# xiexh20/VisTracker

Hardware: AMD Instinct MI355X
Metric: frames/sec joint SMPL+object fit (higher is better)
Workload: dtype f32 (decoder GEMMs: 22-bit split-f16 operands x3 MFMA, fp32 accumulate)

## Files before the change

### include/vistracker.h

```cpp
#ifndef VISTRACKER_H
#define VISTRACKER_H

#ifdef __cplusplus
extern "C" {
#endif

#define VT_OK 0
#define VT_ERR_ARG -1
#define VT_ERR_HIP -2
#define VT_ERR_BUSY -3

#define VT_SMPL_V 6890
#define VT_SMPL_J 52
#define VT_SMPL_NB 10
#define VT_SMPL_NP 459
#define VT_FEAT 611
#define VT_HID 128

const char *vt_last_error(void);
int vt_version(void);

typedef struct vt_smplh vt_smplh;

int vt_smplh_create(vt_smplh **out, const float *v_template, const float *shapedirs, const float *posedirs,
// ... 153 lines not shown

int vt_sqdiff_loss(const float *a, int a_stride, const float *b, int b_stride, int rows, int cols, float denom,
                   float gscale, double *term, float *da, void *stream);

long vt_collision_workspace_bytes(int B, int n_smpl_faces);
int vt_collision_loss(const float *smpl_verts, int n_smpl_verts, const int *smpl_faces, int n_smpl_faces, const float *obj_verts, int n_obj_verts,
                      const int *obj_faces, int n_obj_faces, int B, float sigma, int max_collisions, float gscale, double *term,
                      float *d_obj_t, int *pairs_per_frame, void *workspace, void *stream);

int vt_chamfer_ragged(const float *x, const int *offx, const float *y, const int *offy, int P, float gscale,
                      double *term, float *dx, float *dy, void *stream);
long vt_chamfer_ws_bytes(long total_x, long total_y, int P);
int vt_chamfer_ragged_ws(const float *x, const int *offx, long total_x, const float *y, const int *offy, long total_y, int P, float gscale,
                         double *term, float *dx, float *dy, void *ws, void *stream);

int vt_chamfer_ragged_idx(const float *x, const int *offx, long total_x, const float *y_base, const int *idx_y, const int *offy, long total_y, int P,
                          float gscale, double *term, float *dy_base, void *ws, int run_plan, void *stream);

int vt_nn_distance(const float *query, int nq, const float *search, int ns, int P, float *dist, void *stream);

long vt_sil_workspace_floats(int B, int NV, int NF, int size);
int vt_sil_forward(const float *verts, int B, int NV, const int *faces, int NF, const float *K, int size,
                   float *image, int *face_index, float *ws, void *stream);
int vt_sil_backward(const float *verts, int B, int NV, const int *faces, int NF, const float *K, int size,
                    const int *face_index, const float *d_image, float eps, float *ws, float *dverts, void *stream);
int vt_sil_setup(const float *mask_h, const float *mask_o, int B, int H, int W, const float *crop_centers, double expansion, int out, double crop_size,
                 double net_size, const double *cam_norm, double image_width, float *image_ref, float *keep_mask, float *K, double *boxes_ws, void *stream);

int vt_sil_mask_loss(const float *image, const float *keep, const float *ref, const float *occ, int B, int size,
                     float gscale, double *term, float *per_frame, float *d_image, void *stream);

int vt_sil_step(const float *verts, int B, int NV, const int *faces, int NF, const float *K, int size, const float *keep, const float *ref,
                const float *occ, float gscale, float eps, double *term, int *face_index, float *d_image, float *ws, float *dverts, void *stream);

int vt_triplane_render(const float *verts, const float *center, int B, int NV, const int *faces, int NF, int size,
                       float *masks, int *face_index, float *ws, void *stream);

int vt_upsample2x_bicubic_add(const float *low, const float *skip, int B, int h, int w, int C, float *out, void *stream);
int vt_upsample2x_bicubic_add_stats(const float *low, const float *skip, int B, int h, int w, int C, float *out, double *stats_ws, int stats_groups,
                                    void *stream);

long vt_groupnorm_workspace_doubles(int B, int HW, int C, int groups);
int vt_groupnorm_nhwc(const float *x, const float *gamma, const float *beta, int B, int HW, int C, int groups, float eps,
                      int relu, double *ws, float *y, void *stream);

int vt_adam_step(float *p, const float *g, float *m, float *v, long n, int step, float lr, float beta1, float beta2,
                 float eps, const int *stop_flag, void *stream);

int vt_adam_step_2d(float *p, long p_stride, const float *g, long g_stride, float *m, float *v, int rows, int cols,
                    int step, float lr, float beta1, float beta2, float eps, const int *stop_flag, void *stream);

int vt_loss_reduce_and_stop(const double *terms, const float *w, int nterms, float tol, int armed, float *state,
                            int *stop_flag, float *history, int slot, void *stream);

int vt_fill(float *p, long n, float value, void *stream);

int vt_stream_set_skip_flag(void *stream, const int *flag);

int vt_gen_round_compact(const float *surface, const float *df_target, const float *pre, const unsigned char *active, int B, int S, float filter_val,
                         float zmin, const long long *fill, int cap, int write, float *buf_points, int *order, float *kept_pre, long long *cnt,
                         long long *fill_out, void *stream);
int vt_gen_scatter_heads(const float *pred, int B, int C, int kmax, const long long *fill_old, const long long *cnt, int cap, float *buf, void *stream);
int vt_gen_resample(const float *samples, const int *order, const long long *cnt, const float *init, int B, int S, int S0, const float *u,
                    const float *pert, int M, float near_scale, float *out, void *stream);

long vt_render_workspace_bytes(int B, int NF, int size, int anti_aliasing, long list_entries);
// ... 49 lines not shown
```

### vistracker_amd/_lib.py

```python
from __future__ import annotations

import ctypes as C
import os

_HERE = os.path.dirname(os.path.abspath(__file__))
LIB_PATH = os.environ.get("VT_LIB_PATH", os.path.join(_HERE, "libvistracker_hip.so"))

vp = C.c_void_p
fp = C.c_void_p
ci = C.c_int
cl = C.c_long
cf = C.c_float
cd = C.c_double


class VtMaps(C.Structure):
    _fields_ = [("maps", C.c_void_p * 8), ("res", C.c_int * 8), ("proj", C.c_void_p), ("proj_cols", C.c_int),
                ("act_level", C.c_int), ("proj_level", C.c_int), ("force_fp32", C.c_int)]


SIGNATURES = {
    "vt_last_error": (C.c_char_p, []),
    "vt_version": (ci, []),
    "vt_smplh_create": (ci, [C.POINTER(vp), vp, vp, vp, vp, vp, vp, vp]),
# ... 53 lines not shown
    "vt_conv1x1_destroy": (None, [vp]),
    "vt_conv1x1_forward": (ci, [vp, fp, ci, ci, fp, fp, fp, ci, ci, ci, ci, fp, ci, ci, fp, ci, ci, fp, ci, vp]),
    "vt_conv3x3_forward_block": (ci, [vp, fp, ci, ci, fp, fp, fp, ci, ci, ci, ci, fp, ci, ci, fp, ci, ci, fp, ci, ci, fp, ci, vp]),
    "vt_conv3x3_forward_block_stats": (ci, [vp, fp, ci, ci, fp, fp, fp, ci, ci, ci, ci, fp, ci, ci, fp, ci, ci, fp, ci, ci, fp, ci, fp, ci, vp]),
    "vt_avgpool2x2_stats": (ci, [fp, ci, ci, ci, ci, fp, fp, ci, vp]),
    "vt_sweep_blocks": (ci, [ci]),
    "vt_upsample2x_bicubic_add_stats": (ci, [fp, fp, ci, ci, ci, ci, fp, fp, ci, vp]),
    "vt_conv3x3_forward_gn_stats": (ci, [vp, fp, ci, ci, fp, fp, fp, ci, ci, ci, ci, fp, ci, ci, fp, ci, vp]),
    "vt_triplane_render": (ci, [fp, fp, ci, ci, fp, ci, ci, fp, fp, fp, vp]),
    "vt_query_project_step": (ci, [vp, C.POINTER(VtMaps), fp, fp, fp, ci, ci, ci, cf, fp, fp, vp]),
    "vt_query_projection_floats": (C.c_long, [C.POINTER(VtMaps), ci]),
    "vt_query_build_projection": (ci, [vp, C.POINTER(VtMaps), ci, fp, vp]),
    "vt_so3_project_forward": (ci, [fp, fp, ci, fp, vp]),
    "vt_so3_project_backward": (ci, [fp, fp, ci, fp, fp, vp]),
    "vt_rigid_forward": (ci, [fp, ci, fp, fp, fp, ci, ci, fp, vp]),
    "vt_rigid_backward": (ci, [fp, ci, fp, ci, ci, fp, fp, fp, ci, vp]),
    "vt_accel_loss": (ci, [fp, ci, ci, fp, cf, fp, fp, vp]),
    "vt_accel_loss_strided": (ci, [fp, ci, ci, ci, fp, cf, fp, fp, vp]),
    "vt_velocity_loss": (ci, [fp, ci, ci, cf, fp, fp, vp]),
    "vt_kpts_loss": (ci, [fp, fp, fp, ci, ci, ci, vp, cf, cf, fp, fp, vp]),
    "vt_sqdiff_loss": (ci, [fp, ci, fp, ci, ci, ci, cf, cf, fp, fp, vp]),
    "vt_chamfer_ragged": (ci, [fp, fp, fp, fp, ci, cf, fp, fp, fp, vp]),
    "vt_chamfer_ws_bytes": (C.c_long, [C.c_long, C.c_long, ci]),
    "vt_chamfer_ragged_ws": (ci, [fp, fp, C.c_long, fp, fp, C.c_long, ci, cf, fp, fp, fp, fp, vp]),
    "vt_chamfer_ragged_idx": (ci, [fp, fp, C.c_long, fp, fp, fp, C.c_long, ci, cf, fp, fp, fp, ci, vp]),
    "vt_collision_workspace_bytes": (cl, [ci, ci]),
    "vt_collision_loss": (ci, [fp, ci, fp, ci, fp, ci, fp, ci, ci, cf, ci, cf, fp, fp, fp, fp, vp]),
    "vt_nn_distance": (ci, [fp, ci, fp, ci, ci, fp, vp]),
    "vt_sil_workspace_floats": (cl, [ci, ci, ci, ci]),
    "vt_sil_forward": (ci, [fp, ci, ci, fp, ci, fp, ci, fp, fp, fp, vp]),
    "vt_sil_backward": (ci, [fp, ci, ci, fp, ci, fp, ci, fp, fp, cf, fp, fp, vp]),
    "vt_sil_mask_loss": (ci, [fp, fp, fp, fp, ci, ci, cf, fp, fp, fp, vp]),
    "vt_sil_step": (ci, [fp, ci, ci, fp, ci, fp, ci, fp, fp, fp, cf, cf, fp, fp, fp, fp, fp, vp]),
    "vt_gen_round_compact": (ci, [fp, fp, fp, vp, ci, ci, cf, cf, vp, ci, ci, fp, vp, fp, vp, vp, vp]),
    "vt_gen_scatter_heads": (ci, [fp, ci, ci, ci, vp, vp, ci, fp, vp]),
    "vt_gen_resample": (ci, [fp, vp, vp, fp, ci, ci, ci, fp, fp, ci, cf, fp, vp]),
    "vt_sil_setup": (ci, [fp, fp, ci, ci, ci, fp, C.c_double, ci, C.c_double, C.c_double, C.POINTER(C.c_double), C.c_double, fp, fp, fp, fp, vp]),
    "vt_adam_step": (ci, [fp, fp, fp, fp, cl, ci, cf, cf, cf, cf, fp, vp]),
    "vt_adam_step_2d": (ci, [fp, cl, fp, cl, fp, fp, ci, ci, ci, cf, cf, cf, cf, fp, vp]),
    "vt_loss_reduce_and_stop": (ci, [fp, vp, ci, cf, ci, fp, fp, fp, ci, vp]),
    "vt_fill": (ci, [fp, cl, cf, vp]),
    "vt_selftest_mfma": (ci, [fp, fp, fp, vp]),
    "vt_query_set_clock_probe": (ci, [vp]),
    "vt_render_workspace_bytes": (cl, [ci, ci, ci, ci, cl]),
    "vt_render_static_create": (ci, [C.POINTER(vp), fp, ci, fp, ci, fp, fp, cf, C.POINTER(cf), ci, ci, vp]),
    "vt_render_static_destroy": (None, [vp]),
    "vt_render_rgb": (ci, [fp, ci, ci, fp, ci, fp, fp, ci, cf, C.POINTER(cf), C.POINTER(cf), vp, ci, ci, fp, fp, fp, fp, fp, cl,
                           C.POINTER(cl), vp]),
    "vt_render_panel_u8": (ci, [fp, ci, ci, ci, ci, ci, ci, fp, fp, C.c_longlong, vp]),
    "vt_render_rgb_pv": (ci, [fp, ci, ci, fp, ci, fp, ci, fp, ci, cf, C.POINTER(cf), C.POINTER(cf), vp, ci, ci, fp, fp, fp, fp, fp, cl,
                              C.POINTER(cl), vp]),
    "vt_contact_regions": (ci, [fp, fp, fp, ci, ci, ci, ci, cf, fp, fp, fp, fp, fp, vp]),
    "vt_contact_spheres": (ci, [fp, fp, ci, ci, fp, ci, cf, fp, vp]),
    "vt_contact_face_colors": (ci, [fp, ci, ci, fp, ci, ci, fp, ci, fp, ci, fp, vp]),
    "vt_jpeg_workspace_bytes": (cl, [ci, ci, ci, ci, C.POINTER(C.c_longlong)]),
    "vt_jpeg_encode": (ci, [fp, ci, ci, ci, C.c_longlong, C.c_longlong, ci, ci, vp, cl, vp, C.c_longlong,
                            C.POINTER(C.c_longlong), vp]),
    "vt_mask_bbox": (ci, [fp, fp, ci, ci, ci, ci, fp, vp]),
    "vt_crop_resize_compose": (ci, [fp, fp, fp, ci, ci, ci, fp, ci, ci, fp, fp, C.c_longlong, vp]),
    "vt_resize_panel_u8": (ci, [fp, C.c_longlong, vp, ci, ci, ci, ci, ci, fp, fp, C.c_longlong, vp]),
    "vt_overlay_panel_u8": (ci, [fp, fp, ci, ci, ci, ci, ci, ci, fp, fp, fp, C.c_longlong, cf, vp]),
    "vt_mask_score": (ci, [fp, ci, ci, ci, ci, ci, ci, fp, C.c_longlong, fp, C.c_longlong, vp, ci, fp, vp]),
    "vt_point_mesh_workspace_bytes": (cl, [ci, ci]),
    "vt_point_mesh_distance": (ci, [fp, ci, fp, ci, fp, ci, ci, fp, fp, fp, vp, vp]),
    "vt_point_mesh_distance_ex": (ci, [fp, ci, fp, ci, fp, ci, ci, fp, fp, fp, vp, ci, fp, vp]),
    "vt_nearest_vertex": (ci, [fp, ci, fp, ci, ci, fp, fp, vp]),
# ... 63 lines not shown
```

### vistracker_amd/csrc/sil.hip

```cpp
#include "common.h"

#define SIL_NEAR 0.1f
#define SIL_FAR 100.0f
#define TILE 16
#define MAXLIST 8192

__global__ void sil_project_kernel(const float *__restrict__ verts, const float *__restrict__ K, int NV, float *__restrict__ proj, const int *skip)
{
    VT_SKIP_RETURN(skip);
    const int i = blockIdx.x * blockDim.x + threadIdx.x, b = blockIdx.y;
    if (i >= NV) return;
    const float *v = verts + ((size_t)b * NV + i) * 3, *k = K + 9 * b;
    const float z = v[2], x_ = v[0] / (z + 1e-9f), y_ = v[1] / (z + 1e-9f);
    const float u = k[0] * x_ + k[1] * y_ + k[2];
    const float w = 1.0f - (k[3] * x_ + k[4] * y_ + k[5]);
    float *o = proj + ((size_t)b * NV + i) * 3;
    o[0] = 2.0f * (u - 0.5f); o[1] = 2.0f * (w - 0.5f); o[2] = z;
}

__global__ void sil_triplane_project_kernel(const float *__restrict__ verts, const float *__restrict__ center, int NV, float z_offset,
                                            float *__restrict__ proj)
{
    const int i = blockIdx.x * blockDim.x + threadIdx.x, bv = blockIdx.y, b = bv / 3, view = bv - 3 * b;
    if (i >= NV) return;
    const float *v = verts + ((size_t)b * NV + i) * 3;
    const float x = v[0] - center[3 * b], y = v[1] - center[3 * b + 1], z = v[2] - center[3 * b + 2];
    float *o = proj + ((size_t)bv * NV + i) * 3;
    if (view == 0) { o[0] = z; o[1] = -y; o[2] = -x + z_offset; }
    else if (view == 1) { o[0] = -x; o[1] = -y; o[2] = -z + z_offset; }
    else { o[0] = x; o[1] = z; o[2] = y + z_offset; }
}

__device__ __forceinline__ void load_face(const float *__restrict__ pv, const int *__restrict__ faces, int NF, int f2, float *fc)
{
    const int f = f2 < NF ? f2 : f2 - NF;
    int i0 = faces[3 * f], i1 = faces[3 * f + 1], i2 = faces[3 * f + 2];
    if (f2 >= NF) { const int t = i1; i1 = i2; i2 = t; }
    fc[0] = pv[3 * i0]; fc[1] = pv[3 * i0 + 1]; fc[2] = pv[3 * i0 + 2];
    fc[3] = pv[3 * i1]; fc[4] = pv[3 * i1 + 1]; fc[5] = pv[3 * i1 + 2];
    fc[6] = pv[3 * i2]; fc[7] = pv[3 * i2 + 1]; fc[8] = pv[3 * i2 + 2];
}

#define SIL_FIX 17179869184.0
struct SilWs { unsigned long long *zbuf, *rowmask, *colmask; float *proj, *fc; int2 *fbox; int *visible; double *gproj; unsigned long long *cnt; unsigned *ticket; int *nvis, *vlist; unsigned *ftick; };
static inline SilWs sil_ws(float *ws, int B, int NV, int NF, int is)
{
    SilWs w;
    w.zbuf = reinterpret_cast<unsigned long long *>(ws);
    w.rowmask = w.zbuf + (size_t)B * is * is;
    w.colmask = w.rowmask + (size_t)B * is * (is / 64);
    w.proj = reinterpret_cast<float *>(w.colmask + (size_t)B * is * (is / 64));
    w.fc = w.proj + (size_t)B * NV * 3; w.fbox = reinterpret_cast<int2 *>(w.fc + (size_t)B * 2 * NF * 9);
    w.visible = reinterpret_cast<int *>(w.fbox + (size_t)B * 2 * NF); w.gproj = reinterpret_cast<double *>((reinterpret_cast<uintptr_t>(w.visible + (size_t)B * 2 * NF) + 7) & ~(uintptr_t)7);
    w.cnt = reinterpret_cast<unsigned long long *>(w.gproj + (size_t)B * NV * 2);
    w.ticket = reinterpret_cast<unsigned *>(w.cnt + B);
    w.nvis = reinterpret_cast<int *>(w.ticket + 2);
    w.vlist = w.nvis + B;
    w.ftick = reinterpret_cast<unsigned *>(w.vlist + (size_t)B * NF);
    return w;
}
extern "C" long vt_sil_workspace_floats(int B, int NV, int NF, int size)
{
    return 2L * B * size * size + 4L * B * size * (size / 64) + (long)B * NV * 3 + (long)B * 2 * NF * (9 + 2 + 1) + (long)B * NV * 4 + 16 + 2L * B + 8 + (long)B * (NF + 2);
}

__global__ void sil_face_setup_kernel(const float *__restrict__ proj, const int *__restrict__ faces, int NV, int NF, int is,
                                      float *__restrict__ fcbuf, int2 *__restrict__ fbox, int *__restrict__ visible, const int *skip)
{
    VT_SKIP_RETURN(skip);
    const int f2 = blockIdx.x * blockDim.x + threadIdx.x, b = blockIdx.y;
    if (f2 >= 2 * NF) return;
    float fc[9]; load_face(proj + (size_t)b * NV * 3, faces, NF, f2, fc);
    float *o = fcbuf + ((size_t)b * 2 * NF + f2) * 9;
#pragma unroll
    for (int e = 0; e < 9; e++) o[e] = fc[e];
    visible[(size_t)b * 2 * NF + f2] = 0;
    int x0 = 1, x1 = 0, y0 = 1, y1 = 0;
    if (!((fc[7] - fc[1]) * (fc[3] - fc[0]) < (fc[4] - fc[1]) * (fc[6] - fc[0]))) {
        const float xmin = fminf(fc[0], fminf(fc[3], fc[6])), xmax = fmaxf(fc[0], fmaxf(fc[3], fc[6]));
        const float ymin = fminf(fc[1], fminf(fc[4], fc[7])), ymax = fmaxf(fc[1], fmaxf(fc[4], fc[7]));
        const float fx0 = fminf(fmaxf(floorf((xmin * is + is - 1) * 0.5f) - 1.f, -1.f), (float)is), fx1 = fminf(fmaxf(ceilf((xmax * is + is - 1) * 0.5f) + 1.f, -1.f), (float)is);
        const float fy0 = fminf(fmaxf(floorf((ymin * is + is - 1) * 0.5f) - 1.f, -1.f), (float)is), fy1 = fminf(fmaxf(ceilf((ymax * is + is - 1) * 0.5f) + 1.f, -1.f), (float)is);
        x0 = max((int)fx0, 0); x1 = min((int)fx1, is - 1); y0 = max((int)fy0, 0); y1 = min((int)fy1, is - 1);
        if (y0 > y1) { x0 = 1; x1 = 0; }
    }
    fbox[(size_t)b * 2 * NF + f2] = make_int2((x0 & 0xffff) | (x1 << 16), (y0 & 0xffff) | (y1 << 16));
}

#ifndef SIL_G
#define SIL_G 16
#endif
#ifndef SIL_GS
#define SIL_GS SIL_G
#endif
#define SIL_BIG 128
__device__ __forceinline__ void sil_box_pixel(int p, int x0, int y0, int w, float rw, int &xi, int &yi)
// ... 3 lines not shown
    xi = x0 + r; yi = y0 + q;
}
__device__ __forceinline__ void sil_ndc(int xi, int yi, int is, bool pow2, float ris, float &xp, float &yp)
{
    const float xn = 2.0f * xi + 1 - is, yn = 2.0f * yi + 1 - is;
    xp = pow2 ? xn * ris : xn / is; yp = pow2 ? yn * ris : yn / is;
}
__device__ __forceinline__ bool sil_inside(const float (&fc)[9], float xp, float yp)
{
    return !(((yp - fc[1]) * (fc[3] - fc[0]) < (xp - fc[0]) * (fc[4] - fc[1])) ||
             ((yp - fc[4]) * (fc[6] - fc[3]) < (xp - fc[3]) * (fc[7] - fc[4])) ||
             ((yp - fc[7]) * (fc[0] - fc[6]) < (xp - fc[6]) * (fc[1] - fc[7])));
}
#ifndef SIL_IMG_ABL
#define SIL_IMG_ABL 0
#endif
#ifndef SIL_COMPACT
#define SIL_COMPACT 0
#endif
#ifndef SIL_FAST_Z
#define SIL_FAST_Z 1
#endif
#define SIL_RIM 0.015625f
#ifndef SIL_ZPRETEST
#define SIL_ZPRETEST 0
#endif
__device__ __forceinline__ void sil_zmin(unsigned long long *p, unsigned long long key)
{
#if SIL_ZPRETEST
    if (*(volatile unsigned long long *)p <= key) return;
#endif
    atomicMin(p, key);
}
__device__ __forceinline__ void sil_vote(const float (&fc)[9], float den, int f2, float xp, float yp, int xi, int yi, int is, unsigned long long *__restrict__ zrow)
{
    const float n0 = (fc[4] - fc[7]) * xp + (fc[6] - fc[3]) * yp + (fc[3] * fc[7] - fc[6] * fc[4]);
    const float n1 = (fc[7] - fc[1]) * xp + (fc[0] - fc[6]) * yp + (fc[6] * fc[1] - fc[0] * fc[7]);
    const float n2 = (fc[1] - fc[4]) * xp + (fc[3] - fc[0]) * yp + (fc[0] * fc[4] - fc[3] * fc[1]);
#if SIL_FAST_Z
    {
        const float rden = __builtin_amdgcn_rcpf(den);
        const float a0 = n0 * rden, a1 = n1 * rden, a2 = n2 * rden;
        if (fminf(a0, fminf(a1, a2)) > SIL_RIM && fmaxf(a0, fmaxf(a1, a2)) < 1.0f - SIL_RIM) {
            const float ws_ = a0 + a1 + a2;
            const float zp_ = ws_ * __builtin_amdgcn_rcpf(a0 * __builtin_amdgcn_rcpf(fc[2]) + a1 * __builtin_amdgcn_rcpf(fc[5]) + a2 * __builtin_amdgcn_rcpf(fc[8]));
            if (!(zp_ > SIL_NEAR * 1.001f && zp_ < SIL_FAR * 0.999f)) goto exact;
            sil_zmin(zrow + (size_t)yi * is + xi, ((unsigned long long)__float_as_uint(zp_) << 32) | (unsigned)f2);
            return;
        }
    }
exact:
#endif
    float w0 = n0 / den;
    float w1 = n1 / den;
    float w2 = n2 / den;
    w0 = fminf(fmaxf(w0, 0.f), 1.f); w1 = fminf(fmaxf(w1, 0.f), 1.f); w2 = fminf(fmaxf(w2, 0.f), 1.f);
    const float ws = w0 + w1 + w2;
    const float zp = 1.0f / (w0 / ws / fc[2] + w1 / ws / fc[5] + w2 / ws / fc[8]);
    if (!(zp > SIL_NEAR && zp < SIL_FAR)) return;
    const unsigned long long key = ((unsigned long long)__float_as_uint(zp) << 32) | (unsigned)f2;
    sil_zmin(zrow + (size_t)yi * is + xi, key);
}
__device__ __forceinline__ void sil_scatter_box(const float (&fc)[9], float den, int f2, int x0, int y0, int w, int npx, int start, int stride, int is,
                                                unsigned long long *__restrict__ zrow)
{
    const float rw = 1.0f / (float)w;
    const bool pow2 = (is & (is - 1)) == 0;
    const float ris = 1.0f / (float)is;
    for (int p = start; p < npx; p += stride) {
        int xi, yi; sil_box_pixel(p, x0, y0, w, rw, xi, yi);
        float xp, yp; sil_ndc(xi, yi, is, pow2, ris, xp, yp);
        if (sil_inside(fc, xp, yp)) sil_vote(fc, den, f2, xp, yp, xi, yi, is, zrow);
    }
}
#ifndef SIL_WG_BARRIER
#define SIL_WG_BARRIER 0
#endif
__global__ __launch_bounds__(256) void sil_scatter_kernel(const float *__restrict__ fcbuf, const int2 *__restrict__ fbox, int NF, int is,
                                                          unsigned long long *__restrict__ zbuf, const int *skip)
{
    VT_SKIP_RETURN(skip);
    constexpr int FPW = 64 / SIL_GS;
    __shared__ unsigned short sQ[4][FPW][SIL_BIG];
    const int lane = threadIdx.x & 63, gl = lane % SIL_GS, grp = lane / SIL_GS, b = blockIdx.y;
    const int f = (blockIdx.x * 4 + (threadIdx.x >> 6)) * FPW + grp;
    unsigned long long *zrow = zbuf + (size_t)b * is * is;
    float fc[9]; float den = 0.f; int f2 = 0, x0 = 0, y0 = 0, w = 1, npx = 0;
    if (f < NF) {
        float fa[9];
#pragma unroll
        for (int e = 0; e < 9; e++) fa[e] = fcbuf[((size_t)b * 2 * NF + f) * 9 + e];
        const int2 bbA = fbox[(size_t)b * 2 * NF + f], bbB = fbox[(size_t)b * 2 * NF + NF + f];
        const bool useA = (bbA.x & 0xffff) <= (bbA.x >> 16);
        const int2 bb = useA ? bbA : bbB;
        f2 = useA ? f : f + NF;
        fc[0] = fa[0]; fc[1] = fa[1]; fc[2] = fa[2];
        fc[3] = useA ? fa[3] : fa[6]; fc[4] = useA ? fa[4] : fa[7]; fc[5] = useA ? fa[5] : fa[8];
        fc[6] = useA ? fa[6] : fa[3]; fc[7] = useA ? fa[7] : fa[4]; fc[8] = useA ? fa[8] : fa[5];
        x0 = bb.x & 0xffff; y0 = bb.y & 0xffff;
        const int x1 = bb.x >> 16, y1 = bb.y >> 16;
        den = fc[0] * (fc[4] - fc[7]) + fc[3] * (fc[7] - fc[1]) + fc[6] * (fc[1] - fc[4]);
        if (x0 <= x1 && den != 0.f) { w = x1 - x0 + 1; npx = w * (y1 - y0 + 1); }
    } else {
#pragma unroll
        for (int e = 0; e < 9; e++) fc[e] = 0.f;
    }
    const bool big = npx > SIL_BIG;
    const float rw = 1.0f / (float)w;
    const bool pow2 = (is & (is - 1)) == 0;
    const float ris = 1.0f / (float)is;
    unsigned short *qz = sQ[threadIdx.x >> 6][grp];
    int n_in = 0;
    const int nsmall = big ? 0 : npx;
    for (int p0 = 0; p0 < nsmall; p0 += SIL_GS) {
        const int p = p0 + gl;
        bool in = false;
        if (p < nsmall) {
            int xi, yi; sil_box_pixel(p, x0, y0, w, rw, xi, yi);
            float xp, yp; sil_ndc(xi, yi, is, pow2, ris, xp, yp);
            in = sil_inside(fc, xp, yp);
        }
        const unsigned bits = (unsigned)(__ballot(in) >> (SIL_GS * grp)) & (SIL_GS >= 32 ? 0xffffffffu : ((1u << (SIL_GS & 31)) - 1u));
        if (in) qz[n_in + __popc(bits & ((1u << gl) - 1u))] = (unsigned short)p;
        n_in += __popc(bits);
    }
#if SIL_WG_BARRIER
    __syncthreads();
#else
    __builtin_amdgcn_fence(__ATOMIC_RELEASE, "wavefront");
    __builtin_amdgcn_wave_barrier();
    __builtin_amdgcn_fence(__ATOMIC_ACQUIRE, "wavefront");
#endif
    for (int i = gl; i < n_in; i += SIL_GS) {
        const int p = qz[i];
// ... 230 lines not shown
    o[0] = gx_ / z; o[1] = gy_ / z; o[2] = -(gx_ * v[0] + gy_ * v[1]) / (z * z);
}

__global__ __launch_bounds__(256) void sil_mask_loss_kernel(const float *__restrict__ image, const float *__restrict__ keep, const float *__restrict__ ref,
                                                            const float *__restrict__ occ, int B, int npx, float gs, double *term,
                                                            float *per_frame, float *__restrict__ d_image, const int *skip)
{
    VT_SKIP_RETURN(skip);
    __shared__ double red[4];
    const int b = blockIdx.y;
    const float ob = occ[b];
    double acc = 0;
    const int nq = npx >> 2, per_slice = (nq + gridDim.x - 1) / gridDim.x, i_end = min(nq, (int)(blockIdx.x + 1) * per_slice);
    const float4 *im4 = (const float4 *)(image + (size_t)b * npx), *kp4 = (const float4 *)(keep + (size_t)b * npx), *rf4 = (const float4 *)(ref + (size_t)b * npx);
    float4 *di4 = d_image ? (float4 *)(d_image + (size_t)b * npx) : nullptr;
    for (int i = blockIdx.x * per_slice + threadIdx.x; i < i_end; i += 256) {
        const float4 im = im4[i], kp = kp4[i], rf = rf4[i];
        const float d0 = kp.x * im.x - rf.x, d1 = kp.y * im.y - rf.y, d2 = kp.z * im.z - rf.z, d3 = kp.w * im.w - rf.w;
        acc += (double)(d0 * d0) + (double)(d1 * d1) + (double)(d2 * d2) + (double)(d3 * d3);
        if (di4) di4[i] = make_float4(2.f * d0 * kp.x * ob * gs, 2.f * d1 * kp.y * ob * gs, 2.f * d2 * kp.z * ob * gs, 2.f * d3 * kp.w * ob * gs);
    }
    for (int o = 32; o > 0; o >>= 1) acc += __shfl_xor(acc, o, 64);
    if ((threadIdx.x & 63) == 0) red[threadIdx.x >> 6] = acc;
    __syncthreads();
    if (threadIdx.x == 0) {
        const double per = red[0] + red[1] + red[2] + red[3];
        if (per_frame) per_frame[b] = (float)per;
        if (term) atomicAdd(term, per * (double)ob / (double)B);
    }
}

__global__ void sil_setup_kernel(const float *__restrict__ verts, const float *__restrict__ K, const int *__restrict__ faces, int NV, int NF, int is,
                                 float *__restrict__ fcbuf, int2 *__restrict__ fbox, int *__restrict__ visible, unsigned long long *__restrict__ zbuf,
                                 unsigned long long *__restrict__ cnt, unsigned *__restrict__ ticket, int *__restrict__ nvis, unsigned *__restrict__ ftick, const int *skip)
{
    VT_SKIP_RETURN(skip);
    const int b = blockIdx.y;
    if (blockIdx.x == 0 && threadIdx.x == 0) { cnt[b] = 0ull; nvis[b] = 0; ftick[b] = 0u; if (b == 0) *ticket = 0u; }
    {
        uint4 *z4 = reinterpret_cast<uint4 *>(zbuf + (size_t)b * is * is);
        const int n4 = is * is / 2;
        for (int i = blockIdx.x * blockDim.x + threadIdx.x; i < n4; i += gridDim.x * blockDim.x) z4[i] = make_uint4(~0u, ~0u, ~0u, ~0u);
    }
    const int f2 = blockIdx.x * blockDim.x + threadIdx.x;
    if (f2 >= 2 * NF) return;
    const int f = f2 < NF ? f2 : f2 - NF;
    int vi[3] = {faces[3 * f], faces[3 * f + 1], faces[3 * f + 2]};
    if (f2 >= NF) { const int t = vi[1]; vi[1] = vi[2]; vi[2] = t; }
    const float *k = K + 9 * b;
    float fc[9];
#pragma unroll
    for (int c = 0; c < 3; c++) {
        const float *v = verts + ((size_t)b * NV + vi[c]) * 3;
        const float z = v[2], x_ = v[0] / (z + 1e-9f), y_ = v[1] / (z + 1e-9f);
        const float u = k[0] * x_ + k[1] * y_ + k[2];
        const float w = 1.0f - (k[3] * x_ + k[4] * y_ + k[5]);
        fc[3 * c] = 2.0f * (u - 0.5f); fc[3 * c + 1] = 2.0f * (w - 0.5f); fc[3 * c + 2] = z;
    }
    float *o = fcbuf + ((size_t)b * 2 * NF + f2) * 9;
#pragma unroll
    for (int e = 0; e < 9; e++) o[e] = fc[e];
    visible[(size_t)b * 2 * NF + f2] = 0;
    int x0 = 1, x1 = 0, y0 = 1, y1 = 0;
    if (!((fc[7] - fc[1]) * (fc[3] - fc[0]) < (fc[4] - fc[1]) * (fc[6] - fc[0]))) {
        const float xmin = fminf(fc[0], fminf(fc[3], fc[6])), xmax = fmaxf(fc[0], fmaxf(fc[3], fc[6]));
        const float ymin = fminf(fc[1], fminf(fc[4], fc[7])), ymax = fmaxf(fc[1], fmaxf(fc[4], fc[7]));
        const float fx0 = fminf(fmaxf(floorf((xmin * is + is - 1) * 0.5f) - 1.f, -1.f), (float)is), fx1 = fminf(fmaxf(ceilf((xmax * is + is - 1) * 0.5f) + 1.f, -1.f), (float)is);
        const float fy0 = fminf(fmaxf(floorf((ymin * is + is - 1) * 0.5f) - 1.f, -1.f), (float)is), fy1 = fminf(fmaxf(ceilf((ymax * is + is - 1) * 0.5f) + 1.f, -1.f), (float)is);
        x0 = max((int)fx0, 0); x1 = min((int)fx1, is - 1); y0 = max((int)fy0, 0); y1 = min((int)fy1, is - 1);
        if (y0 > y1) { x0 = 1; x1 = 0; }
    }
    fbox[(size_t)b * 2 * NF + f2] = make_int2((x0 & 0xffff) | (x1 << 16), (y0 & 0xffff) | (y1 << 16));
}

__global__ __launch_bounds__(256) void sil_image_kernel(const unsigned long long *__restrict__ zbuf, int NV, int NF, int is, const float *__restrict__ keep,
                                                        const float *__restrict__ ref, const float *__restrict__ occ, int B, float gs, double *term,
                                                        int *__restrict__ face_index, float *__restrict__ d_image, float *__restrict__ image, int *__restrict__ visible,
                                                        unsigned long long *__restrict__ rowmask, unsigned long long *__restrict__ colmask, double *__restrict__ gproj,
                                                        unsigned long long *__restrict__ cnt, unsigned *__restrict__ ticket, int *__restrict__ nvis,
                                                        int *__restrict__ vlist, unsigned *__restrict__ ftick, const int *skip)
{
    VT_SKIP_RETURN(skip);
    __shared__ unsigned sCol[4][64];
    __shared__ double sSum[4];
    const int lane = threadIdx.x & 63, wave = threadIdx.x >> 6, wpl = is / 64;
    const int tile = blockIdx.x, b = blockIdx.y, tiles = wpl * wpl;
    const int tx = tile % wpl, ty = tile / wpl;
    const int xi = tx * 64 + lane;
    {
        unsigned long long *g = reinterpret_cast<unsigned long long *>(gproj) + (size_t)b * NV * 2;
        if (!(SIL_IMG_ABL & 4)) for (int i = tile * 256 + threadIdx.x; i < NV * 2; i += tiles * 256) g[i] = 0ull;
    }
    const float ob = occ[b];
    unsigned long long key[16]; float kp[16], rf[16];
#pragma unroll
    for (int r = 0; r < 16; r++) {
        const int yi = ty * 64 + wave * 16 + r;
        const size_t o = ((size_t)b * is + (is - 1 - yi)) * is + xi;
        key[r] = zbuf[((size_t)b * is + yi) * is + xi]; kp[r] = keep[o]; rf[r] = ref[o];
    }
    constexpr int LCAP = 1024;
    __shared__ int sList[LCAP];
    __shared__ int sN, sBase;
    if (threadIdx.x == 0) sN = 0;
    __syncthreads();
    int fown[16], seen[16];
#pragma unroll
    for (int r = 0; r < 16; r++) {
        fown[r] = key[r] == ~0ull ? -1 : (int)(unsigned)(key[r] & 0xffffffffull);
        seen[r] = (SIL_COMPACT && fown[r] >= 0) ? visible[(size_t)b * 2 * NF + fown[r]] : 1;
    }
    unsigned col = 0; double acc = 0;
#pragma unroll
    for (int r = 0; r < 16; r++) {
        const int yi = ty * 64 + wave * 16 + r;
        const size_t o = ((size_t)b * is + (is - 1 - yi)) * is + xi;
        const int f = fown[r];
        const float im = f >= 0 ? 1.0f : 0.0f;
        face_index[o] = f;
        if (image) image[o] = im;
#if SIL_COMPACT
        const int f_left = __shfl_up(f, 1, 64);
        const bool rim = (lane == 0 || f_left != f) && (r == 0 || fown[r > 0 ? r - 1 : 0] != f);
        if (seen[r] == 0 && rim && atomicExch(visible + (size_t)b * 2 * NF + f, 1) == 0) {
            const int k = atomicAdd(&sN, 1);
            if (k < LCAP) sList[k] = f; else vlist[(size_t)b * NF + atomicAdd(nvis + b, 1)] = f;
        }
#else
#if !(SIL_IMG_ABL & 2)
        if (f >= 0) visible[(size_t)b * 2 * NF + f] = 1;
#endif
#endif
        const float d = kp[r] * im - rf[r];
        acc += (double)(d * d);
        const float gd = 2.f * d * kp[r] * ob * gs;
        d_image[o] = gd;
        const bool p = f < 0 && gd < 0.f;
        const unsigned long long m = __ballot(p);
        if (lane == 0 && !(SIL_IMG_ABL & 8)) rowmask[((size_t)b * is + yi) * wpl + tx] = m;
        col |= (unsigned)p << r;
    }
    sCol[wave][lane] = col;
    for (int o_ = 32; o_ > 0; o_ >>= 1) acc += __shfl_xor(acc, o_, 64);
    if (lane == 0) sSum[wave] = acc;
    __syncthreads();
    {
        const int nl = min(sN, LCAP);
        if (threadIdx.x == 0 && nl > 0) sBase = atomicAdd(nvis + b, nl);
        __syncthreads();
        for (int i = threadIdx.x; i < nl; i += 256) vlist[(size_t)b * NF + sBase + i] = sList[i];
    }
    if (wave == 0)
        colmask[((size_t)b * is + xi) * wpl + ty] = (unsigned long long)sCol[0][lane] | ((unsigned long long)sCol[1][lane] << 16) |
                                                     ((unsigned long long)sCol[2][lane] << 32) | ((unsigned long long)sCol[3][lane] << 48);
    if (threadIdx.x == 0 && !(SIL_IMG_ABL & 1)) atomicAdd(cnt + b, (unsigned long long)__double2ll_rn((sSum[0] + sSum[1] + sSum[2] + sSum[3]) * SIL_FIX));
}

extern "C" int vt_sil_step(const float *verts, int B, int NV, const int *faces, int NF, const float *K, int size, const float *keep, const float *ref,
                           const float *occ, float gscale, float eps, double *term, int *face_index, float *d_image, float *ws, float *dverts, void *stream)
{
    VT_REQUIRE(verts && faces && K && keep && ref && occ && face_index && d_image && ws && dverts && B > 0 && NV > 0 && NF > 0 && size > 0 && size % 64 == 0 && size < 32768,
               "vt_sil_step: bad argument (size must be a multiple of 64)");
    hipStream_t st = vt_stream(stream); const int *skip = vt_skip_flag_of(st);
    const SilWs w = sil_ws(ws, B, NV, NF, size);
    hipLaunchKernelGGL(sil_setup_kernel, dim3((2 * NF + 255) / 256, B), dim3(256), 0, st, verts, K, faces, NV, NF, size, w.fc, w.fbox, w.visible, w.zbuf, w.cnt, w.ticket, w.nvis, w.ftick, skip);
    VT_LAUNCH_CHECK();
    hipLaunchKernelGGL(sil_scatter_kernel, dim3((NF + 4 * (64 / SIL_GS) - 1) / (4 * (64 / SIL_GS)), B), dim3(256), 0, st, w.fc, w.fbox, NF, size, w.zbuf, skip);
    VT_LAUNCH_CHECK();
    hipLaunchKernelGGL(sil_image_kernel, dim3((size / 64) * (size / 64), B), dim3(256), 0, st, w.zbuf, NV, NF, size, keep, ref, occ, B, gscale / (float)B, term, face_index,
                       d_image, (float *)nullptr, w.visible, w.rowmask, w.colmask, w.gproj, w.cnt, w.ticket, w.nvis, w.vlist, w.ftick, skip);
    VT_LAUNCH_CHECK();
    hipLaunchKernelGGL(sil_bwd_face_kernel, dim3((NF + 4 * (64 / SIL_G) - 1) / (4 * (64 / SIL_G)), B), dim3(256), 0, st, w.fc, w.visible, faces, NV, NF, size, face_index, d_image,
                       w.rowmask, w.colmask, eps, w.gproj, SIL_COMPACT ? w.nvis : (const int *)nullptr, SIL_COMPACT ? w.vlist : (const int *)nullptr, skip);
    VT_LAUNCH_CHECK();
    hipLaunchKernelGGL(sil_unproject_kernel, dim3((NV + 255) / 256, B), dim3(256), 0, st, verts, K, NV, w.gproj, dverts, w.cnt, occ, B, term, skip);
    VT_LAUNCH_CHECK();
    return VT_OK;
}

extern "C" int vt_sil_forward(const float *verts, int B, int NV, const int *faces, int NF, const float *K, int size, float *image,
                              int *face_index, float *ws, void *stream)
{
    VT_REQUIRE(verts && faces && K && image && face_index && ws && B > 0 && NV > 0 && NF > 0 && size > 0 && size % TILE == 0 && size < 32768,
               "vt_sil_forward: bad argument (size must be a multiple of 64)");
    VT_REQUIRE(size % 64 == 0, "vt_sil_forward: size must be a multiple of 64");
    hipStream_t st = vt_stream(stream); const int *skip = vt_skip_flag_of(st);
    const SilWs w = sil_ws(ws, B, NV, NF, size);
    hipLaunchKernelGGL(sil_project_kernel, dim3((NV + 255) / 256, B), dim3(256), 0, st, verts, K, NV, w.proj, skip);
    VT_LAUNCH_CHECK();
    hipLaunchKernelGGL(sil_face_setup_kernel, dim3((2 * NF + 255) / 256, B), dim3(256), 0, st, w.proj, faces, NV, NF, size, w.fc, w.fbox, w.visible, skip);
    VT_LAUNCH_CHECK();
    VT_HIP(hipMemsetAsync(w.zbuf, 0xff, sizeof(unsigned long long) * (size_t)B * size * size, st));
    hipLaunchKernelGGL(sil_scatter_kernel, dim3((NF + 4 * (64 / SIL_GS) - 1) / (4 * (64 / SIL_GS)), B), dim3(256), 0, st, w.fc, w.fbox, NF, size, w.zbuf, skip);
    VT_LAUNCH_CHECK();
    hipLaunchKernelGGL(sil_resolve_kernel, dim3((size + 255) / 256, size, B), dim3(256), 0, st, w.zbuf, NF, size, image, face_index, w.visible, skip);
    VT_LAUNCH_CHECK();
    return VT_OK;
}

extern "C" int vt_triplane_render(const float *verts, const float *center, int B, int NV, const int *faces, int NF, int size, float *masks,
                                  int *face_index, float *ws, void *stream)
{
    VT_REQUIRE(verts && center && faces && masks && face_index && ws && B > 0 && NV > 0 && NF > 0 && size > 0 && size % 64 == 0 && size < 32768,
// ... 134 lines not shown
```

Before: 152.1.

## Bin faces into 64x64 tiles and rasterize z-buffer in shared memory

Silhouette rasterization now bins each face's bounding box into per-tile lists during setup, then the image kernel rasterizes each 64x64 tile's faces into a shared-memory depth buffer with LDS atomicMin. This drops the global z-buffer clear, the separate scatter kernel and the global 64-bit atomics. The cost is extra global atomics for binning, a memset of the tile counters, and a fallback that scans every face for any tile whose list overflows the cap. Shared-memory use in the image kernel rises sharply, which can reduce occupancy.

```diff
diff --git a/include/vistracker.h b/include/vistracker.h
--- a/include/vistracker.h
+++ b/include/vistracker.h
@@ -209,6 +209,7 @@
 
 int vt_sil_step(const float *verts, int B, int NV, const int *faces, int NF, const float *K, int size, const float *keep, const float *ref,
                 const float *occ, float gscale, float eps, double *term, int *face_index, float *d_image, float *ws, float *dverts, void *stream);
+int vt_sil_tile_capacity(void);
 
 int vt_triplane_render(const float *verts, const float *center, int B, int NV, const int *faces, int NF, int size,
                        float *masks, int *face_index, float *ws, void *stream);
diff --git a/vistracker_amd/_lib.py b/vistracker_amd/_lib.py
--- a/vistracker_amd/_lib.py
+++ b/vistracker_amd/_lib.py
@@ -109,6 +109,7 @@
     "vt_sil_backward": (ci, [fp, ci, ci, fp, ci, fp, ci, fp, fp, cf, fp, fp, vp]),
     "vt_sil_mask_loss": (ci, [fp, fp, fp, fp, ci, ci, cf, fp, fp, fp, vp]),
     "vt_sil_step": (ci, [fp, ci, ci, fp, ci, fp, ci, fp, fp, fp, cf, cf, fp, fp, fp, fp, fp, vp]),
+    "vt_sil_tile_capacity": (ci, []),
     "vt_gen_round_compact": (ci, [fp, fp, fp, vp, ci, ci, cf, cf, vp, ci, ci, fp, vp, fp, vp, vp, vp]),
     "vt_gen_scatter_heads": (ci, [fp, ci, ci, ci, vp, vp, ci, fp, vp]),
     "vt_gen_resample": (ci, [fp, vp, vp, fp, ci, ci, ci, fp, fp, ci, cf, fp, vp]),
diff --git a/vistracker_amd/csrc/sil.hip b/vistracker_amd/csrc/sil.hip
--- a/vistracker_amd/csrc/sil.hip
+++ b/vistracker_amd/csrc/sil.hip
@@ -42,7 +42,18 @@
 }
 
 #define SIL_FIX 17179869184.0
-struct SilWs { unsigned long long *zbuf, *rowmask, *colmask; float *proj, *fc; int2 *fbox; int *visible; double *gproj; unsigned long long *cnt; unsigned *ticket; int *nvis, *vlist; unsigned *ftick; };
+#ifndef SIL_TILES
+#define SIL_TILES 1
+#endif
+#ifndef SIL_TILE_CAP
+#define SIL_TILE_CAP 2048
+#endif
+#ifndef SIL_TSTAGE
+#define SIL_TSTAGE 128
+#endif
+static inline int sil_tile_cap(int NF) { return NF < SIL_TILE_CAP ? NF : SIL_TILE_CAP; }
+extern "C" int vt_sil_tile_capacity(void) { return SIL_TILES ? SIL_TILE_CAP : 0; }
+struct SilWs { unsigned long long *zbuf, *rowmask, *colmask; float *proj, *fc; int2 *fbox; int *visible; double *gproj; unsigned long long *cnt; unsigned *ticket; int *nvis, *vlist; unsigned *ftick; int *tcnt, *tlist; };
 static inline SilWs sil_ws(float *ws, int B, int NV, int NF, int is)
 {
     SilWs w;
@@ -57,11 +68,14 @@
     w.nvis = reinterpret_cast<int *>(w.ticket + 2);
     w.vlist = w.nvis + B;
     w.ftick = reinterpret_cast<unsigned *>(w.vlist + (size_t)B * NF);
+    w.tcnt = reinterpret_cast<int *>(w.ftick + B);
+    w.tlist = w.tcnt + (size_t)B * (is / 64) * (is / 64);
     return w;
 }
 extern "C" long vt_sil_workspace_floats(int B, int NV, int NF, int size)
 {
-    return 2L * B * size * size + 4L * B * size * (size / 64) + (long)B * NV * 3 + (long)B * 2 * NF * (9 + 2 + 1) + (long)B * NV * 4 + 16 + 2L * B + 8 + (long)B * (NF + 2);
+    return 2L * B * size * size + 4L * B * size * (size / 64) + (long)B * NV * 3 + (long)B * 2 * NF * (9 + 2 + 1) + (long)B * NV * 4 + 16 + 2L * B + 8 + (long)B * (NF + 2) +
+           (SIL_TILES ? (long)B * (size / 64) * (size / 64) * (sil_tile_cap(NF) + 1) : 0L);
 }
 
 __global__ void sil_face_setup_kernel(const float *__restrict__ proj, const int *__restrict__ faces, int NV, int NF, int is,
@@ -131,7 +145,11 @@
 #endif
     atomicMin(p, key);
 }
-__device__ __forceinline__ void sil_vote(const float (&fc)[9], float den, int f2, float xp, float yp, int xi, int yi, int is, unsigned long long *__restrict__ zrow)
+__device__ __forceinline__ float sil_den(const float (&fc)[9])
+{
+    return fc[0] * (fc[4] - fc[7]) + fc[3] * (fc[7] - fc[1]) + fc[6] * (fc[1] - fc[4]);
+}
+__device__ __forceinline__ bool sil_pixel_key(const float (&fc)[9], float den, int f2, float xp, float yp, unsigned long long &key)
 {
     const float n0 = (fc[4] - fc[7]) * xp + (fc[6] - fc[3]) * yp + (fc[3] * fc[7] - fc[6] * fc[4]);
     const float n1 = (fc[7] - fc[1]) * xp + (fc[0] - fc[6]) * yp + (fc[6] * fc[1] - fc[0] * fc[7]);
@@ -144,8 +162,8 @@
             const float ws_ = a0 + a1 + a2;
             const float zp_ = ws_ * __builtin_amdgcn_rcpf(a0 * __builtin_amdgcn_rcpf(fc[2]) + a1 * __builtin_amdgcn_rcpf(fc[5]) + a2 * __builtin_amdgcn_rcpf(fc[8]));
             if (!(zp_ > SIL_NEAR * 1.001f && zp_ < SIL_FAR * 0.999f)) goto exact;
-            sil_zmin(zrow + (size_t)yi * is + xi, ((unsigned long long)__float_as_uint(zp_) << 32) | (unsigned)f2);
-            return;
+            key = ((unsigned long long)__float_as_uint(zp_) << 32) | (unsigned)f2;
+            return true;
         }
     }
 exact:
@@ -156,9 +174,14 @@
     w0 = fminf(fmaxf(w0, 0.f), 1.f); w1 = fminf(fmaxf(w1, 0.f), 1.f); w2 = fminf(fmaxf(w2, 0.f), 1.f);
     const float ws = w0 + w1 + w2;
     const float zp = 1.0f / (w0 / ws / fc[2] + w1 / ws / fc[5] + w2 / ws / fc[8]);
-    if (!(zp > SIL_NEAR && zp < SIL_FAR)) return;
-    const unsigned long long key = ((unsigned long long)__float_as_uint(zp) << 32) | (unsigned)f2;
-    sil_zmin(zrow + (size_t)yi * is + xi, key);
+    if (!(zp > SIL_NEAR && zp < SIL_FAR)) return false;
+    key = ((unsigned long long)__float_as_uint(zp) << 32) | (unsigned)f2;
+    return true;
+}
+__device__ __forceinline__ void sil_vote(const float (&fc)[9], float den, int f2, float xp, float yp, int xi, int yi, int is, unsigned long long *__restrict__ zrow)
+{
+    unsigned long long key;
+    if (sil_pixel_key(fc, den, f2, xp, yp, key)) sil_zmin(zrow + (size_t)yi * is + xi, key);
 }
 __device__ __forceinline__ void sil_scatter_box(const float (&fc)[9], float den, int f2, int x0, int y0, int w, int npx, int start, int stride, int is,
                                                 unsigned long long *__restrict__ zrow)
@@ -198,7 +221,7 @@
         fc[6] = useA ? fa[6] : fa[3]; fc[7] = useA ? fa[7] : fa[4]; fc[8] = useA ? fa[8] : fa[5];
         x0 = bb.x & 0xffff; y0 = bb.y & 0xffff;
         const int x1 = bb.x >> 16, y1 = bb.y >> 16;
-        den = fc[0] * (fc[4] - fc[7]) + fc[3] * (fc[7] - fc[1]) + fc[6] * (fc[1] - fc[4]);
+        den = sil_den(fc);
         if (x0 <= x1 && den != 0.f) { w = x1 - x0 + 1; npx = w * (y1 - y0 + 1); }
     } else {
 #pragma unroll
@@ -495,12 +518,13 @@
 
 __global__ void sil_setup_kernel(const float *__restrict__ verts, const float *__restrict__ K, const int *__restrict__ faces, int NV, int NF, int is,
                                  float *__restrict__ fcbuf, int2 *__restrict__ fbox, int *__restrict__ visible, unsigned long long *__restrict__ zbuf,
-                                 unsigned long long *__restrict__ cnt, unsigned *__restrict__ ticket, int *__restrict__ nvis, unsigned *__restrict__ ftick, const int *skip)
+                                 unsigned long long *__restrict__ cnt, unsigned *__restrict__ ticket, int *__restrict__ nvis, unsigned *__restrict__ ftick,
+                                 int *__restrict__ tcnt, int *__restrict__ tlist, int cap, const int *skip)
 {
     VT_SKIP_RETURN(skip);
     const int b = blockIdx.y;
     if (blockIdx.x == 0 && threadIdx.x == 0) { cnt[b] = 0ull; nvis[b] = 0; ftick[b] = 0u; if (b == 0) *ticket = 0u; }
-    {
+    if (!SIL_TILES) {
         uint4 *z4 = reinterpret_cast<uint4 *>(zbuf + (size_t)b * is * is);
         const int n4 = is * is / 2;
         for (int i = blockIdx.x * blockDim.x + threadIdx.x; i < n4; i += gridDim.x * blockDim.x) z4[i] = make_uint4(~0u, ~0u, ~0u, ~0u);
@@ -534,6 +558,17 @@
         if (y0 > y1) { x0 = 1; x1 = 0; }
     }
     fbox[(size_t)b * 2 * NF + f2] = make_int2((x0 & 0xffff) | (x1 << 16), (y0 & 0xffff) | (y1 << 16));
+#if SIL_TILES
+    if (x0 <= x1 && (f2 < NF || ((fc[4] - fc[1]) * (fc[6] - fc[0]) < (fc[7] - fc[1]) * (fc[3] - fc[0])))) {
+        const int wpl = is / 64, tiles = wpl * wpl;
+        for (int ty = y0 >> 6; ty <= (y1 >> 6); ty++)
+            for (int tx = x0 >> 6; tx <= (x1 >> 6); tx++) {
+                const size_t t = (size_t)b * tiles + ty * wpl + tx;
+                const int k = atomicAdd(tcnt + t, 1);
+                if (k < cap) tlist[t * cap + k] = f2;
+            }
+    }
+#endif
 }
 
 __global__ __launch_bounds__(256) void sil_image_kernel(const unsigned long long *__restrict__ zbuf, int NV, int NF, int is, const float *__restrict__ keep,
@@ -541,7 +576,8 @@
                                                         int *__restrict__ face_index, float *__restrict__ d_image, float *__restrict__ image, int *__restrict__ visible,
                                                         unsigned long long *__restrict__ rowmask, unsigned long long *__restrict__ colmask, double *__restrict__ gproj,
                                                         unsigned long long *__restrict__ cnt, unsigned *__restrict__ ticket, int *__restrict__ nvis,
-                                                        int *__restrict__ vlist, unsigned *__restrict__ ftick, const int *skip)
+                                                        int *__restrict__ vlist, unsigned *__restrict__ ftick, const float *__restrict__ fcbuf,
+                                                        const int2 *__restrict__ fbox, const int *__restrict__ tcnt, const int *__restrict__ tlist, int cap, const int *skip)
 {
     VT_SKIP_RETURN(skip);
     __shared__ unsigned sCol[4][64];
@@ -556,13 +592,79 @@
     }
     const float ob = occ[b];
     unsigned long long key[16]; float kp[16], rf[16];
+#if SIL_TILES
+    __shared__ unsigned long long sKey[64 * 64];
+    __shared__ float sRec[12][SIL_TSTAGE];
+    {
+        const int nb = tcnt[(size_t)b * tiles + tile];
+        const bool ovf = nb > cap;
+        const int n = ovf ? 2 * NF : nb;
+        if (n > 0) {
+            const int *list = tlist + ((size_t)b * tiles + tile) * cap;
+            const size_t fb = (size_t)b * 2 * NF;
+            float rc[9]; int2 rb; int rf2;
+            auto fetch = [&](int i) {
+                rb = make_int2(1, 0); rf2 = 0;
+#pragma unroll
+                for (int e = 0; e < 9; e++) rc[e] = 0.f;
+                if (i < n) {
+                    const int f2 = ovf ? i : list[i];
+                    rb = fbox[fb + f2]; rf2 = f2;
+                    if (ovf && f2 >= NF) { const int2 ba = fbox[fb + f2 - NF]; if ((ba.x & 0xffff) <= (ba.x >> 16)) rb = make_int2(1, 0); }
+#pragma unroll
+                    for (int e = 0; e < 9; e++) rc[e] = fcbuf[(fb + f2) * 9 + e];
+                }
+            };
+            if (threadIdx.x < SIL_TSTAGE) fetch(threadIdx.x);
+            for (int i = threadIdx.x; i < 64 * 64; i += 256) sKey[i] = ~0ull;
+            const int grp = threadIdx.x >> 4, gl = threadIdx.x & 15;
+            const bool pow2 = (is & (is - 1)) == 0;
+            const float ris = 1.0f / (float)is;
+            for (int c0 = 0; c0 < n; c0 += SIL_TSTAGE) {
+                if (threadIdx.x < SIL_TSTAGE) {
+#pragma unroll
+                    for (int e = 0; e < 9; e++) sRec[e][threadIdx.x] = rc[e];
+                    sRec[9][threadIdx.x] = __int_as_float(rb.x); sRec[10][threadIdx.x] = __int_as_float(rb.y); sRec[11][threadIdx.x] = __int_as_float(rf2);
+                }
+                __syncthreads();
+                if (c0 + SIL_TSTAGE < n && threadIdx.x < SIL_TSTAGE) fetch(c0 + SIL_TSTAGE + threadIdx.x);
+                const int m = min(SIL_TSTAGE, n - c0);
+                for (int j = grp; j < m; j += 16) {
+                    const int bx = __float_as_int(sRec[9][j]), by = __float_as_int(sRec[10][j]);
+                    const int x0 = max(bx & 0xffff, tx * 64), x1 = min(bx >> 16, tx * 64 + 63), y0 = max(by & 0xffff, ty * 64), y1 = min(by >> 16, ty * 64 + 63);
+                    if (x0 > x1 || y0 > y1) continue;
+                    float fc[9];
+#pragma unroll
+                    for (int e = 0; e < 9; e++) fc[e] = sRec[e][j];
+                    const float den = sil_den(fc);
+                    if (den == 0.f) continue;
+                    const int f2 = __float_as_int(sRec[11][j]);
+                    const int w = x1 - x0 + 1, npx = w * (y1 - y0 + 1);
+                    const float rw = 1.0f / (float)w;
+                    for (int p = gl; p < npx; p += 16) {
+                        int px, py; sil_box_pixel(p, x0, y0, w, rw, px, py);
+                        float xp, yp; sil_ndc(px, py, is, pow2, ris, xp, yp);
+                        unsigned long long k_;
+                        if (sil_inside(fc, xp, yp) && sil_pixel_key(fc, den, f2, xp, yp, k_)) atomicMin(&sKey[(py - ty * 64) * 64 + (px - tx * 64)], k_);
+                    }
+                }
+                __syncthreads();
+            }
+        }
+#pragma unroll
+        for (int r = 0; r < 16; r++) key[r] = n > 0 ? sKey[(wave * 16 + r) * 64 + lane] : ~0ull;
+    }
+#endif
 #pragma unroll
     for (int r = 0; r < 16; r++) {
         const int yi = ty * 64 + wave * 16 + r;
         const size_t o = ((size_t)b * is + (is - 1 - yi)) * is + xi;
-        key[r] = zbuf[((size_t)b * is + yi) * is + xi]; kp[r] = keep[o]; rf[r] = ref[o];
-    }
-    constexpr int LCAP = 1024;
+#if !SIL_TILES
+        key[r] = zbuf[((size_t)b * is + yi) * is + xi];
+#endif
+        kp[r] = keep[o]; rf[r] = ref[o];
+    }
+    constexpr int LCAP = SIL_COMPACT ? 1024 : 1;
     __shared__ int sList[LCAP];
     __shared__ int sN, sBase;
     if (threadIdx.x == 0) sN = 0;
@@ -626,12 +728,19 @@
                "vt_sil_step: bad argument (size must be a multiple of 64)");
     hipStream_t st = vt_stream(stream); const int *skip = vt_skip_flag_of(st);
     const SilWs w = sil_ws(ws, B, NV, NF, size);
-    hipLaunchKernelGGL(sil_setup_kernel, dim3((2 * NF + 255) / 256, B), dim3(256), 0, st, verts, K, faces, NV, NF, size, w.fc, w.fbox, w.visible, w.zbuf, w.cnt, w.ticket, w.nvis, w.ftick, skip);
-    VT_LAUNCH_CHECK();
+    const int cap = sil_tile_cap(NF);
+#if SIL_TILES
+    VT_HIP(hipMemsetAsync(w.tcnt, 0, sizeof(int) * (size_t)B * (size / 64) * (size / 64), st));
+#endif
+    hipLaunchKernelGGL(sil_setup_kernel, dim3((2 * NF + 255) / 256, B), dim3(256), 0, st, verts, K, faces, NV, NF, size, w.fc, w.fbox, w.visible, w.zbuf, w.cnt, w.ticket, w.nvis, w.ftick,
+                       w.tcnt, w.tlist, cap, skip);
+    VT_LAUNCH_CHECK();
+#if !SIL_TILES
     hipLaunchKernelGGL(sil_scatter_kernel, dim3((NF + 4 * (64 / SIL_GS) - 1) / (4 * (64 / SIL_GS)), B), dim3(256), 0, st, w.fc, w.fbox, NF, size, w.zbuf, skip);
     VT_LAUNCH_CHECK();
+#endif
     hipLaunchKernelGGL(sil_image_kernel, dim3((size / 64) * (size / 64), B), dim3(256), 0, st, w.zbuf, NV, NF, size, keep, ref, occ, B, gscale / (float)B, term, face_index,
-                       d_image, (float *)nullptr, w.visible, w.rowmask, w.colmask, w.gproj, w.cnt, w.ticket, w.nvis, w.vlist, w.ftick, skip);
+                       d_image, (float *)nullptr, w.visible, w.rowmask, w.colmask, w.gproj, w.cnt, w.ticket, w.nvis, w.vlist, w.ftick, w.fc, w.fbox, w.tcnt, w.tlist, cap, skip);
     VT_LAUNCH_CHECK();
     hipLaunchKernelGGL(sil_bwd_face_kernel, dim3((NF + 4 * (64 / SIL_G) - 1) / (4 * (64 / SIL_G)), B), dim3(256), 0, st, w.fc, w.visible, faces, NV, NF, size, face_index, d_image,
                        w.rowmask, w.colmask, eps, w.gproj, SIL_COMPACT ? w.nvis : (const int *)nullptr, SIL_COMPACT ? w.vlist : (const int *)nullptr, skip);
```

Measured after the change: 131.5. 0.864x the previous value.
